# divortio/divortio-lz4

Hardware: AMD Instinct MI355X
Metric: LZ4 compress+decompress GB/s on 4 MiB independent blocks; % of HBM peak (higher is better)
Workload: dtype u8; 1 GPU; raw block decompress, 4096 x 4 MiB independent blocks per GPU (tiles216), device-resident (BASELINE.json configs[1]); blocks_per_gpu=4096, block_bytes=4194304, generator=tiles216, parallelism=blocks sharded x1

## Files before the change

### divortio-lz4_amd/csrc/lz4mi_decompress.hip

```cpp
#include "../../include/lz4mi.h"
#include "lz4mi_common.h"
#include "lz4mi_decompress.h"
#include "lz4mi_launch.h"

#ifndef LZ4MI_LL_ADAPT
#define LZ4MI_LL_ADAPT 127
#endif
#ifndef LZ4MI_ORDER
#define LZ4MI_ORDER 1
#endif
#ifndef LZ4MI_ABLATE
#define LZ4MI_ABLATE 0
#endif

#ifndef LZ4MI_TIMELINE
#define LZ4MI_TIMELINE 0
#endif

#ifndef LZ4MI_PROFILE
#define LZ4MI_PROFILE 0
#endif

namespace lz4mi {

// ... 686 lines not shown
        for (int k = lane; 16 * k < e0 - s0 + 20; k += kWave) {
            const int32_t q = s0 + 16 * k;
            uint4 v;
            if (q + 16 <= per) {
                v = load16<R_HIST>(c, S, R.src + q);
            } else {
                unsigned __int128 x = 0;
#pragma unroll 1
                for (int j = 0; j < 16; ++j) x |= (unsigned __int128)src[(q + j) % per] << (8 * j);
                __builtin_memcpy(&v, &x, 16);
            }
            B.w[4 * k] = v.x;
            B.w[4 * k + 1] = v.y;
            B.w[4 * k + 2] = v.z;
            B.w[4 * k + 3] = v.w;
        }
        __syncthreads();
        const int32_t a0 = (int32_t)((0u - (uint32_t)(uintptr_t)(c.dst + R.y)) & 15u);
        if (lane == 0 && a0) {
            const int32_t ph = 0 - s0;
            if ((uint32_t)ph < (uint32_t)(e0 - s0)) out16(c.dst + R.y, stage16(B.w, ph));
        }
        const int32_t np = (R.n - a0 + 15) >> 4;
        const int32_t step = (16 * kWave) % per;
        int32_t r = (a0 + 16 * lane) % per;
#pragma unroll 2
        for (int32_t p = lane; p < np; p += kWave) {
            const int32_t d0 = a0 + 16 * p;
            const bool last = d0 > dl;
            const int32_t d = last ? dl : d0;
            const int32_t ph = (last ? d % per : r) - s0;
            if ((uint32_t)ph < (uint32_t)(e0 - s0) && LZ4MI_ABLATE != 4) {
                out16(c.dst + R.y + d, stage16(B.w, ph));
            }
            r += step;
            if (r >= per) r -= per;
        }
    }
    __syncthreads();
}


__device__ __forceinline__ void long_literals(uint8_t* dst, const uint8_t* src, int32_t n, int lane) {
    const int32_t np = (n + 15) >> 4;
    auto at = [&](int32_t p) { return 16 * p < n - 16 ? 16 * p : n - 16; };
#if LZ4MI_LL_ADAPT
    const unsigned int* lat = &g_lat_active[32 * xcc_id()];
#endif
    for (int32_t p0 = lane; p0 < np; p0 += kWave * 4) {
#if LZ4MI_LL_ADAPT
        const uint32_t busy = __hip_atomic_load(lat, __ATOMIC_RELAXED, __HIP_MEMORY_SCOPE_AGENT);
#endif
        const int32_t d0 = at(p0), d1 = at(p0 + kWave), d2 = at(p0 + 2 * kWave), d3 = at(p0 + 3 * kWave);
        uint4 v0, v1, v2, v3;
        v0 = ld16_nt(src + d0);
        v1 = ld16_nt(src + d1);
        v2 = ld16_nt(src + d2);
        v3 = ld16_nt(src + d3);
        st16_nt(dst + d0, v0);
        st16_nt(dst + d1, v1);
        st16_nt(dst + d2, v2);
        st16_nt(dst + d3, v3);
#if LZ4MI_LL_ADAPT
        if (busy) __builtin_amdgcn_s_sleep(LZ4MI_LL_ADAPT);
#endif
    }
}

__device__ __forceinline__ void wave_run(const Ctx& c, DecShared& S, int lane, const Run& R, PatBuf B) {
    if (R.kind == R_NONE || R.n <= 0) return;
    const bool in_buf = R.kind == R_HIST || (R.kind == R_BYTES && c.out_off + R.src >= 0);
    if (in_buf && R.period && R.n > kPeriodBulk &&
        B.bytes > 0 && (R.period + 48 <= B.bytes || (R.n >= 4 * R.period && B.bytes >= 1024))) {
        periodic_run(c, S, lane, R, B);
        return;
    }
    const int np = run_pieces(R.n);
    if (R.kind == R_BYTES) {
        for (int p = lane; p < np; p += kWave) {
            const Piece P = plan_piece(R, p);
            bytes_piece(c, P.y, P.a, P.b, P.w, P.period);
        }
        return;
    }
    if (R.period) {
        WaveGen<kWaveB2> g{R, np, 0, lane};
        pipe<R_HIST, true, kWaveB2>(c, S, g);
        return;
    }
    WaveGen<kWaveB> g{R, np, 0, lane};
    if (R.kind == R_LDS) pipe<R_LDS, false, kWaveB>(c, S, g);
    else if (R.kind == R_COMP && R.n >= kLongLit) long_literals(c.dst + R.y, c.blk + R.src, R.n, lane);
    else if (R.kind == R_COMP) pipe<R_COMP, false, kWaveB>(c, S, g);
    else pipe<R_HIST, false, kWaveB>(c, S, g);
}

__device__ __forceinline__ void short_literals(const Ctx& c, int32_t y, int32_t n, const uint4& v) {
    if (LZ4MI_ABLATE == 4) return;
    uint8_t* d = c.dst + y;
    uint64_t lo = v.x | ((uint64_t)v.y << 32);
    const uint64_t hi = v.z | ((uint64_t)v.w << 32);
    int32_t o = 0;
    if (n & 8) { __builtin_memcpy(d, &lo, 8); lo = hi; o = 8; }
    if (n & 4) { const uint32_t t = (uint32_t)lo; __builtin_memcpy(d + o, &t, 4); lo >>= 32; o += 4; }
    if (n & 2) { const uint16_t t = (uint16_t)lo; __builtin_memcpy(d + o, &t, 2); lo >>= 16; o += 2; }
    if (n & 1) d[o] = (uint8_t)lo;
}

constexpr int kLitRuns = 64;
constexpr int kLitRows = kLitRuns * (kLaneBytes / 16) / 64;
static_assert((kChunk + 16) / 17 <= kLitRuns, "every run of >= 16 literal bytes of a chunk has a list entry");
static_assert(kLim / 16 + kLitRuns <= 3 * 64, "a chunk's own runs: at most three piece rows");
static_assert(kLim / 16 + kLitRuns <= kLitRows * 64, "... which the bitmap holds");
static_assert(kLitRuns * sizeof(PEnt) + kLitRows * 8 <= sizeof(uint32_t) * kMaxSeq, "run list and bitmap fit S.pms");
static_assert(kLitRows <= kWave, "one lane clears each bitmap word");
static_assert(offsetof(DecShared, pms) % 16 == 0, "16-byte aligned list entries");

struct LitDeal {
    uint32_t P = 0, R = 0;
    static __device__ __forceinline__ PEnt* list(DecShared& S) { return reinterpret_cast<PEnt*>(S.pms); }
    static __device__ __forceinline__ uint64_t* bitmap(DecShared& S) {
        return reinterpret_cast<uint64_t*>(reinterpret_cast<uint8_t*>(S.pms) + kLitRuns * sizeof(PEnt));
    }
    __device__ __forceinline__ void add(DecShared& S, int lane, bool has, uint64_t bal, int32_t y, int32_t src, int32_t n) {
        if (R == 0) {
            if (lane < kLitRows) bitmap(S)[lane] = 0;
            __syncthreads();
        }
        const uint32_t np = has ? (uint32_t)(n + 15) >> 4 : 0u;
        const uint32_t incl = wave_incl_scan(np, lane);
        const uint32_t r = R + __builtin_amdgcn_mbcnt_hi((uint32_t)(bal >> 32), __builtin_amdgcn_mbcnt_lo((uint32_t)bal, 0u));
        const uint32_t p0 = P + incl - np;
        if (has) {
            list(S)[r] = PEnt{y, src, n, (int32_t)p0};
            atomicOr((unsigned long long*)&bitmap(S)[p0 >> 6], 1ull << (p0 & 63u));
        }
        P += lane_of(incl, kWave - 1);
        R += (uint32_t)__popcll(bal);
    }
    __device__ __forceinline__ void flush(const Ctx& c, DecShared& S, int lane) {
        if (R == 0) return;
        __syncthreads();
        const PEnt* L = list(S);
        const uint64_t* bm = bitmap(S);
        int32_t rb = -1;
        for (uint32_t t = 0; 64u * t < P; ++t) {
            const uint64_t w = bm[t];
            const int32_t below = (int32_t)__builtin_amdgcn_mbcnt_hi((uint32_t)(w >> 32), __builtin_amdgcn_mbcnt_lo((uint32_t)w, 0u));
            const int32_t r = rb + below + (int32_t)((w >> lane) & 1u);
            rb += __popcll(w);
            const uint32_t p = 64u * t + (uint32_t)lane;
            if (p < P) {
                const PEnt e = L[r];
                const int32_t d0 = 16 * ((int32_t)p - e.p0);
                const int32_t d = d0 < e.n - 16 ? d0 : e.n - 16;
                const uint4 v = stage16(S.stage, e.src + d);
                if (LZ4MI_ABLATE != 4) out16(c.dst + e.y + d, v);
            }
        }
        __syncthreads();
        P = R = 0;
    }
};

__device__ __forceinline__ void dealt_literals(const Ctx& c, DecShared& S, int lane, uint32_t nseq) {
    LitDeal D;
    for (uint32_t i = 0; 64 * i < nseq; ++i) {
        const uint32_t k = 64 * i + lane;
        const uint4& e = S.t_seq[k < nseq ? k : 0u];
        const uint32_t y = e.x, lw = e.y;
        const uint32_t n = k < nseq ? lw >> 16 : 0u;
        const bool has = n >= 16;
        const uint64_t bal = __ballot(has);
        if (bal) D.add(S, lane, has, bal, (int32_t)y, (int32_t)(lw & 0xFFFFu), (int32_t)n);
    }
    D.flush(c, S, lane);
}

__device__ __forceinline__ int64_t wave_varint(const Ctx& c, int lane, int64_t& q) {
    int64_t sum = 0;
    for (;;) {
        int64_t p = q + 16 * lane;
        int first = 16;
        uint32_t lastb = 0;
        for (int j = 0; j < 16; ++j) {
            int64_t r = p + j;
            uint32_t b = (r < c.in_len) ? c.blk[r] : 0u;
            if (b != 255u && first == 16) { first = j; lastb = b; }
        }
        uint64_t mask = __ballot(first < 16);
        if (mask) {
            int fl = __builtin_ctzll(mask);
            int fi = lane_of(first, fl);
            uint32_t fb = lane_of(lastb, fl);
            int64_t cnt = (int64_t)fl * 16 + fi;
            sum += 255 * cnt + fb;
            q += cnt + 1;
            return sum;
        }
        sum += 255 * 16 * kWave;
        q += 16 * kWave;
    }
}

__device__ __forceinline__ uint32_t seq_error(const Ctx& c, int64_t out_start, int64_t lit, int64_t ll, uint32_t off,
                                              int64_t ml) {
    if (out_start + ll > c.cap) return 1;
    if (lit + ll > c.in_len) return 2;
    if (ml == 0) return 0;
    if (off == 0) return 3;
    int64_t ms_abs = c.out_off + out_start + ll;
    if ((int64_t)off > ms_abs + c.dict_len) return 4;
    if (c.isolate && (int64_t)off > out_start + ll) return 5;
    return 0;
}

__device__ __forceinline__ int32_t err_status(uint32_t e) { return e == 5 ? -9 : -(int32_t)e; }
template <bool XP>
__device__ __forceinline__ uint32_t seq_err(const Ctx& c, bool rel, int64_t out_start, int64_t lit, int64_t ll,
                                            uint32_t off, int64_t ml) {
    if (XP && rel) {
        if (lit + ll > c.in_len) return 2;
        if (ml == 0) return 0;
        return off == 0 ? 3u : 0u;
    }
    return seq_error(c, out_start, lit, ll, off, ml);
}

__device__ __forceinline__ uint32_t f1_changes(const Ctx& c, int32_t ms, int32_t off, int32_t ml) {
    if (ml == 0 || ml >= 8 || off < 8 || c.out_off + ms - off < 0) return 0;
    const int32_t p0 = ms + ml - 8;
    if (p0 - off < 0) return c.isolate ? 2u : 1u;
    for (int32_t p = p0; p < ms && p < c.cap; ++p)
        if (hist_u8(c.dst + p) != hist_u8(c.dst + p - off)) return 1;
    return 0;
}

__device__ __noinline__ void f1_fixup(const Ctx c, const DecShared& S, int lane, uint32_t nseq, bool cut, int64_t cut_ms,
                         int32_t coff, int32_t cml) {
    int64_t lo = INT64_MAX;
    const uint32_t n = nseq + (cut ? 1u : 0u);
    for (uint32_t k = 0; k < n; ++k) {
        int64_t ms;
        int32_t off, ml;
        if (k < nseq) {
            const SeqInfo q = seq_info(S, k);
            ms = (int64_t)q.out + q.ll;
            off = q.off;
            ml = q.ml;
        } else {
            ms = cut_ms;
            off = coff;
            ml = cml;
        }
        if (ml == 0) continue;
        const bool internal = c.out_off + ms - off >= 0;
        if (ms - off + ml > lo) {
            if (internal) {
                for (int32_t t = lane; t < ml; t += kWave) {
                    const int64_t d = ms + t;
                    const int64_t s = ms - off + (off < ml ? t % off : t);
                    const uint32_t v = hist_u8(c.dst + s);
                    if (d < c.cap) c.dst[d] = (uint8_t)v;
                }
            } else if (lane == 0) {
                for (int32_t t = 0; t < ml; ++t) {
                    const uint32_t v = hist_byte(c, ms - off + t);
                    if (ms + t < c.cap) c.dst[ms + t] = (uint8_t)v;
                }
            }
            wait_vmem();
        }
        if (internal && off >= 8 && ml < 8) {
            const int64_t p = ms + ml - 8 + lane;
            const bool mine = lane < 8 - ml && c.out_off + p >= 0 && p < c.cap;
            const uint32_t v = mine ? (c.out_off + p - off >= 0 ? hist_u8(c.dst + p - off) : 0u) : 0u;
            if (mine) c.dst[p] = (uint8_t)v;
            const int64_t p0 = ms + ml - 8;
            if (p0 < lo) lo = p0;
            wait_vmem();
        }
    }
}

__device__ __forceinline__ int32_t stored_block(const DecArgs& a, const Ctx& c, uint32_t b, uint32_t out_cap, int lane) {
    int32_t status = 0;
    const int32_t n = c.in_len;
    if ((uint32_t)n > out_cap) {
        status = LZ4MI_ERR_RANGE_STATUS;
    } else if (n >= 16) {
        long_literals(c.dst, c.blk, n, lane);
    } else if (lane < n) {
        c.dst[lane] = c.blk[lane];
    }
    if (lane == 0) {
        a.status[b] = status;
        a.out_len[b] = status ? 0u : (uint32_t)n;
    }
    return status;
}

struct XState {
    bool on = false;
    uint4* xs = nullptr;
    SegRec* xr = nullptr;
    uint32_t seg_lo = 0, seg_hi = 0;
    bool started = false, done = false, fail = false;
    uint32_t G = 0, X = 0, nx = 0, olen = 0, err = 0xFFFFFFFFu, entry = 0;
    int64_t OG = 0;
    int pass = 0, restart = 0;
};

template <bool LK>
__device__ __forceinline__ bool x_enter(const DecArgs& a, Ctx& c, XState& x, int lane, uint32_t wblk, uint32_t sg,
                                        uint32_t nseg, uint32_t out_cap) {
    x.on = LK || ((uint32_t)c.in_len <= a.x_in_max && out_cap <= a.x_out_max &&
                  (uint64_t)out_cap < (uint64_t)c.in_len * kXRatioMax &&
                  !(a.x_flat1 && (uint64_t)c.in_len * 16 >= (uint64_t)out_cap * 15));
    if (!x.on) return a.xphase == 0 && sg == wblk % nseg;
    const SegGeom G = seg_geom((uint32_t)c.in_len);
    if (sg >= G.S) return false;
    x.seg_lo = sg * G.L;
    x.seg_hi = sg + 1 == G.S ? (uint32_t)c.in_len : min((uint32_t)c.in_len, x.seg_lo + G.L);
    x.xs = a.xseq + (size_t)wblk * a.xseq_stride + (size_t)sg * G.stride;
    x.xr = a.xrec + (size_t)wblk * nseg + sg;
    SegRec* const xr = x.xr;
    if (a.xphase == 2) {
// ... 287 lines not shown
        if (k < nseq) {
            const SeqInfo q = seq_info(S, k);
            e = seq_err<XP>(c, rel, c.O + (uint32_t)(q.out - (int32_t)c.O), (int64_t)c.ip + q.lit, q.ll, q.off, q.ml);
        }
        first_err = wave_min(e ? (k << 3) | e : 0xFFFFFFFFu);
    }
    return SeqTable{nseq, (int64_t)carry, first_err, false};
}

struct CutSeq {
    int64_t cq = 0, cll = 0, cml = 0, clit = 0;
    uint32_t coff = 0;
};

__device__ __forceinline__ void advance(Ctx& c, int64_t tab_hi, const Parse& P, const CutSeq& cs) {
    c.O = tab_hi;
    if (P.cut) {
        c.O += cs.cll + cs.cml;
        c.ip = (int32_t)(cs.cq < c.in_len ? cs.cq : c.in_len);
    } else if (P.tail >= kEnd) {
        c.ip = c.in_len;
    } else {
        c.ip += (int32_t)P.tail;
    }
}

__device__ __forceinline__ void x_export_chunk(Ctx& c, const DecShared& S, XState& x, int lane, const Parse& P,
                                               const SeqTable& T, const CutSeq& cs) {
    const bool cut = P.cut;
    const uint32_t nseq = T.nseq, seg_lo = x.seg_lo, seg_hi = x.seg_hi;
    const int64_t tab_hi = c.O + T.total;
    const uint32_t ipc = (uint32_t)c.ip;
    const uint32_t ntot = nseq + (cut ? 1u : 0u);
    const uint32_t ecut = cut ? seq_err<true>(c, true, tab_hi, cs.clit, cs.cll, cs.coff, cs.cml) : 0u;
    const uint32_t ferr = T.first_err != 0xFFFFFFFFu ? T.first_err : (ecut ? ((nseq << 3) | ecut) : 0xFFFFFFFFu);
    const uint32_t fk = ferr == 0xFFFFFFFFu ? ntot : (ferr >> 3);
    auto x_tok = [&](uint32_t k) -> uint32_t {
        if (k >= nseq) return ipc + P.last_tok;
        const SeqInfo q = seq_info(S, k);
        return ipc + (uint32_t)q.lit - 1u - (q.ll >= 15 ? (uint32_t)(q.ll - 15) / 255u + 1u : 0u);
    };
    auto x_out = [&](uint32_t k) -> int64_t { return k >= nseq ? tab_hi : (int64_t)S.t_seq[k].x; };
    uint32_t k0 = ntot, k1 = ntot;
    for (uint32_t r = 0; 64u * r < ntot; ++r) {
        const uint32_t k = 64u * r + lane;
        const uint32_t t = k < ntot ? x_tok(k) : 0xFFFFFFFFu;
        const uint64_t m0 = __ballot(k < ntot && t >= seg_lo), m1 = __ballot(k < ntot && t >= seg_hi);
        if (k0 == ntot && m0) k0 = 64u * r + (uint32_t)__builtin_ctzll(m0);
        if (k1 == ntot && m1) k1 = 64u * r + (uint32_t)__builtin_ctzll(m1);
    }
    bool restart = false;
    if (!x.started && fk < k0) {
        if (x.pass == 0 && x.restart < kSegRestarts) {
            restart = true;
            ++x.restart;
        } else {
            x.fail = x.done = true;
        }
    } else {
        if (!x.started && k0 < ntot) {
            x.started = true;
            x.G = x_tok(k0);
            x.OG = x_out(k0);
        }
        if (x.started) {
            const uint32_t ke = fk < k1 ? fk + 1 : k1;
            for (uint32_t k = k0 + lane; k < ke; k += kWave) {
                uint4 e;
                if (k < nseq) {
                    const SeqInfo q = seq_info(S, k);
                    e = make_uint4((uint32_t)(x_out(k) - x.OG), ipc + (uint32_t)q.lit, (uint32_t)q.ll,
                                   q.ml ? (uint32_t)q.off : 0u);
                } else {
                    e = make_uint4((uint32_t)(tab_hi - x.OG), (uint32_t)cs.clit, (uint32_t)cs.cll,
                                   cs.cml ? cs.coff : 0u);
                }
                x.xs[x.nx + (k - k0)] = e;
            }
            if (fk < k1) {
                x.err = ((x.nx + (fk - k0)) << 3) | (ferr & 7u);
                x.done = true;
            } else if (k1 < ntot) {
                x.done = true;
                x.X = x_tok(k1);
                x.olen = (uint32_t)(x_out(k1) - x.OG);
            }
            x.nx += ke - k0;
        }
    }
    if (restart) {
        c.ip = (int32_t)(x_tok(fk) + 1u);
        c.O = 0;
    } else if (!x.done) {
        advance(c, tab_hi, P, cs);
        if ((uint32_t)c.ip >= seg_hi && c.ip < c.in_len) {
            if (!x.started) {
                x.started = true;
                x.G = (uint32_t)c.ip;
                x.OG = c.O;
            }
            x.done = true;
            x.X = (uint32_t)c.ip;
            x.olen = (uint32_t)(c.O - x.OG);
        }
    }
    __syncthreads();
}

__device__ __forceinline__ void x_finish(const DecArgs& a, const Ctx& c, XState& x, int lane, uint32_t sg) {
    if (!x.done) {
        if (!x.started) {
            x.G = (uint32_t)c.in_len;
            x.OG = c.O;
        }
        x.X = (uint32_t)c.in_len;
        x.olen = (uint32_t)(c.O - x.OG);
    }
    if (lane == 0) {
        SegRec* const xr = x.xr;
        xr->entry = x.G;
        xr->exit = x.X;
        xr->cnt = x.nx;
        xr->olen = x.olen;
        xr->err = x.err;
        xr->fail = (x.fail || (a.xforce && sg > 0 && (a.xforce == 2 ? x.pass != 1 : x.pass == 0))) ? 1u : 0u;
        if (x.pass == 1)
            __hip_atomic_store(&xr->fin, (x.err != 0xFFFFFFFFu ? kFinErr : x.X) + 1u, __ATOMIC_RELEASE,
                               __HIP_MEMORY_SCOPE_AGENT);
    }
}

__device__ __forceinline__ uint32_t source_map(const Ctx& c, DecShared& S, int lane, uint32_t nseq, int64_t total) {
    uint32_t msh = total >= 32u * nseq ? 5u : 4u;
    while ((total >> msh) >= kLim) ++msh;
    for (uint32_t k = lane; k < nseq; k += kWave) {
        const uint32_t t0 = S.t_seq[k].x - (uint32_t)c.O;
        const uint32_t t1 = (k + 1 < nseq ? S.t_seq[k + 1].x : (uint32_t)(c.O + total)) - (uint32_t)c.O;
        for (uint32_t b = (t0 + (1u << msh) - 1) >> msh; (b << msh) < t1; ++b) S.nxt[b] = (uint16_t)k;
    }
    __syncthreads();
    return msh;
}

__device__ __forceinline__ uint32_t round1(const Ctx& c, DecShared& S, int lane, uint32_t nseq, uint32_t msh, Prof& prof) {
    uint32_t pend = 0;
    uint32_t ready = 0;
    uint32_t rbits = 0;
    uint32_t nlit_pack = 0;
    dealt_literals(c, S, lane, nseq);
    LitDeal D;
    for (uint32_t i = 0; 64 * i < nseq; ++i) {
        const uint32_t k = 64 * i + lane;
        Run M = no_run(), ML = no_run();
        SeqInfo q = seq_info(S, k < nseq ? k : 0u);
        if (k >= nseq) q.ll = 0;
        {
            const bool shortL = q.ll > 0 && q.ll < 16;
            if (__ballot(shortL)) {
                if (shortL) short_literals(c, q.out, q.ll, stage16(S.stage, q.lit));
            }
        }
        PROF(23);
        if (k < nseq) {
            const int32_t t0 = q.out;
            M = match_run(c, t0 + q.ll, q.off, q.ml);
            if (M.n == 0) {
                M.kind = R_NONE;
            } else if (match_src_end(M) > (int32_t)c.O) {
                int32_t rs = M.src, re = match_src_end(M), li = 0, nl = 0;
                const int r = (M.kind == R_HIST && M.period == 0)
                                  ? remap_src(c, S, nseq, msh, rs, re, li, nl, i < 4)
                                  : 0;
                if (r == 3) {
                    ML = Run{M.y, nl, li, 0, R_LDS};
                    M.y += nl;
                    M.n -= nl;
                    nlit_pack |= (uint32_t)nl << (8 * i);
                }
                if (r == 1 || r == 3) {
                    M.src = rs;
                    if (c.out_off + rs < 16) M.kind = R_BYTES;
                    S.t_seq[k].w = (uint32_t)rs + (r == 3 ? kSplitBase : kMemoBase);
                    rbits |= 1u << i;
                } else if (r == 2) {
                    ML = Run{M.y, M.n, li, 0, R_LDS};
                    M.kind = R_NONE;
                } else {
                    pend |= 1u << i;
                    M.kind = R_NONE;
                }
            }
        }
        const bool longM = M.kind != R_NONE && M.n > kLaneBytes;
        const bool longML = ML.n > kLaneBytes;
        const bool fastM = M.kind == R_HIST && M.period == 0 && M.n >= 16;
        if (M.kind != R_NONE && !longM && fastM) ready |= 1u << i;
        PROF(16);
        {
            const bool dealML = ML.n >= 16 && !longML, shortML = ML.n > 0 && ML.n < 16;
            if (const uint64_t bal = __ballot(dealML)) {
                if (D.R + (uint32_t)__popcll(bal) > (uint32_t)kLitRuns) D.flush(c, S, lane);
                D.add(S, lane, dealML, bal, ML.y, ML.src, ML.n);
            }
            if (__ballot(shortML)) {
                if (shortML) short_literals(c, ML.y, ML.n, stage16(S.stage, ML.src));
            }
        }
        PROF(17);
        for (uint64_t lm = __ballot(longML); lm; lm &= lm - 1) wave_run(c, S, lane, shfl_run(ML, __builtin_ctzll(lm)), no_pat());
        if (M.kind != R_NONE && !longM && !fastM) lane_slow_run(c, S, M);
        if (const uint64_t mm0 = __ballot(longM)) {
            D.flush(c, S, lane);
            for (uint64_t mm = mm0; mm; mm &= mm - 1) wave_run(c, S, lane, shfl_run(M, __builtin_ctzll(mm)), pat_round1(S));
        }
        PROF(18);
    }
    D.flush(c, S, lane);
    piece_pipe(c, S, ready, rbits, lane, nseq, nlit_pack);
    return pend;
}

__device__ __forceinline__ void later_rounds(const Ctx& c, DecShared& S, int lane, uint32_t nseq, uint32_t pend,
                                             Prof& prof) {
    for (; LZ4MI_ABLATE != 6;) {
        uint32_t np = 0;
        for (uint32_t i = 0; 64 * i < nseq; ++i) {
            const bool pk = (pend >> i) & 1u;
            const uint64_t bal = __ballot(pk);
            if (pk) {
                const uint32_t k = 64 * i + lane;
                const uint32_t idx = np + __builtin_amdgcn_mbcnt_hi((uint32_t)(bal >> 32),
                                                                    __builtin_amdgcn_mbcnt_lo((uint32_t)bal, 0u));
                const SeqInfo q = seq_info(S, k);
                const int32_t ms = q.out + q.ll;
                S.pms[idx] = (uint32_t)ms;
                S.pme[idx] = (uint32_t)(q.ml > c.cap - ms ? c.cap : ms + q.ml);
            }
            np += (uint32_t)__popcll(bal);
        }
        if (np == 0) break;
        PROF_COUNT(11, 1);
        __syncthreads();
        wait_vmem();
        PROF(20);
        uint32_t ready = 0;
        for (uint32_t i = 0; 64 * i < nseq; ++i) {
            if (__ballot((pend >> i) & 1u) == 0) continue;
            Run M = no_run();
            if ((pend >> i) & 1u) {
                const uint32_t k = 64 * i + lane;
                const SeqInfo q = seq_info(S, k);
                M = match_run(c, q.out + q.ll, q.off, q.ml);
                const int32_t rs = M.src, re = match_src_end(M);
                uint32_t lo = 0, hi = np;
                while (lo < hi) {
                    const uint32_t mid = (lo + hi) >> 1;
                    if ((int32_t)S.pme[mid] > rs) hi = mid;
                    else lo = mid + 1;
                }
                if (lo >= np || (int32_t)S.pms[lo] >= re) pend &= ~(1u << i);
                else M.kind = R_NONE;
            }
            const bool longM = M.kind != R_NONE && M.n > kLaneBytes;
            const bool fastM = M.kind == R_HIST && M.period == 0 && M.n >= 16;
            if (M.kind != R_NONE && !longM && fastM) ready |= 1u << i;
            if (M.kind != R_NONE && !longM && !fastM) lane_slow_run(c, S, M);
            for (uint64_t mm = __ballot(longM); mm; mm &= mm - 1) wave_run(c, S, lane, shfl_run(M, __builtin_ctzll(mm)), pat_rounds(S));
        }
        piece_pipe(c, S, ready, 0u, lane, nseq, 0u);
        __syncthreads();
    }
}

__device__ __forceinline__ void output_rounds(const Ctx& c, DecShared& S, int lane, const SeqTable& T, Prof& prof) {
    const uint32_t msh = source_map(c, S, lane, T.nseq, T.total);
    PROF(22);
    const uint32_t pend = round1(c, S, lane, T.nseq, msh, prof);
    PROF(19);
    later_rounds(c, S, lane, T.nseq, pend, prof);
}

__device__ __forceinline__ int32_t f1_table(const Ctx& c, const DecShared& S, int lane, uint32_t nseq) {
    bool cand = false;
    for (uint32_t k = lane; k < nseq; k += kWave) {
        const SeqInfo q = seq_info(S, k);
        cand |= q.ml != 0 && q.ml < 8 && q.off >= 8;
    }
    if (__ballot(cand)) {
        wait_vmem();
        uint32_t dv = 0;
        for (uint32_t k = lane; k < nseq; k += kWave) {
            const SeqInfo q = seq_info(S, k);
            dv |= f1_changes(c, q.out + q.ll, q.off, q.ml);
        }
        if (__ballot(dv & 2u)) return -9;
        if (__ballot(dv)) f1_fixup(c, S, lane, nseq, false, 0, 0, 0);
    }
    return 0;
}

__device__ __forceinline__ int32_t cut_match(const Ctx& c, DecShared& S, int lane, int32_t ms, const CutSeq& cs,
                                             bool f1check) {
    const Run M = match_run(c, ms, (int32_t)cs.coff, (int32_t)cs.cml);
    if (M.n > 0) {
        wait_vmem();
        wave_run(c, S, lane, M, pat_all(S));
    }
    if (f1check && cs.cml != 0 && cs.cml < 8 && cs.coff >= 8) {
        wait_vmem();
        const uint32_t dv = lane == 0 ? f1_changes(c, ms, (int32_t)cs.coff, (int32_t)cs.cml) : 0u;
        if (__ballot(dv & 2u)) return -9;
        if (__ballot(dv)) f1_fixup(c, S, lane, 0, true, (int64_t)ms, (int32_t)cs.coff, (int32_t)cs.cml);
    }
    return 0;
}

constexpr bool kOutput = LZ4MI_ABLATE == 0 || LZ4MI_ABLATE >= 4;
constexpr bool kParseOnly = LZ4MI_ABLATE == 2 || LZ4MI_ABLATE == 3;

template <bool XP, bool LK = false, bool CH = false>
__device__ __forceinline__ int32_t decompress_block(const DecArgs& a, uint32_t cblk = 0, uint64_t cbase = 0) {
    __shared__ DecShared S;
    const int lane = threadIdx.x;
    const uint32_t nseg = XP ? a.xsegs : 1u;
    if (!CH && blockIdx.x >= a.nblocks * nseg) return 0;
    const uint32_t wblk = CH ? cblk : XP ? blockIdx.x / nseg : blockIdx.x;
    const uint32_t sg = XP ? blockIdx.x - wblk * nseg : 0u;
    if (LK && uniform(a.xcnt[wblk]) == kNotExported) return 0;
    const uint32_t b = CH ? cblk : a.order ? uniform(a.order[wblk]) : wblk;
    if (!CH && !XP && a.redo && !uniform(a.redo[b])) return 0;
#if LZ4MI_TIMELINE
    const uint64_t tl_t0 = wall_clock64();
#endif
    const uint64_t in_off = uniform64(a.in_off[b]), out_off = uniform64(a.out_off[b]);
    const uint32_t out_cap = uniform(a.out_cap[b]);
    Ctx c;
    c.blk = a.in + in_off;
    const uint32_t word = uniform(a.in_len[b]);
    c.in_len = (int32_t)(a.frame_words ? word & 0x7FFFFFFFu : word);
    c.out_off = CH ? (int64_t)(out_off - cbase) : (int64_t)out_off;
    c.dst = a.out + out_off;
    c.cap = out_cap > 0x7FFFFFFFu ? 0x7FFFFFFF : (int32_t)out_cap;
    c.dict = a.dict;
    c.dict_len = a.dict ? (int32_t)a.dict_len : 0;
    c.isolate = a.isolate;
    c.ip = 0;
    c.O = 0;
    if (a.frame_words && (word & 0x80000000u)) {
        return stored_block(a, c, b, out_cap, lane);
    }
    XState x;
    if constexpr (XP) {
        if (!x_enter<LK>(a, c, x, lane, wblk, sg, nseg, out_cap)) return 0;
    }
    const bool xp = XP && x.on;
#if LZ4MI_LL_ADAPT
    const bool lat_bound = (uint64_t)c.in_len * 2 < (uint64_t)out_cap;
    unsigned int* lat = &g_lat_active[32 * xcc_id()];
    if (lat_bound && lane == 0) atomicAdd(lat, 1u);
#endif
    Prefetch pf;
    Prof prof;
#if LZ4MI_PROFILE
    prof = Prof{{0}, (uint64_t)wall_clock64()};
#endif
    int32_t status = 0;
    while (c.ip < c.in_len) {
        if (XP && x.done) break;
        PROF_COUNT(10, 1);
        stage_chunk(c, S, pf, lane);
        const uint32_t rem = (uint32_t)(c.in_len - c.ip);
        Parse P;
        SeqTable T;
        for (bool fast_tab = rem > kFastRem;; fast_tab = false) {
            P = parse_chunk(S, lane, rem, fast_tab, !XP, prof);
            if (LZ4MI_ABLATE != 3 && !P.cut && P.tail < kEnd && (int64_t)c.ip + P.tail < c.in_len)
                prefetch(c, pf, (int64_t)c.ip + P.tail, lane);
            if (kParseOnly) break;
            T = seq_table<XP>(c, S, lane, rem, xp, fast_tab, P, prof);
            if (!T.redo) break;
            wait_vmem();
            settle(pf);
            __syncthreads();
        }
        if (kParseOnly) {
            c.ip = P.tail == kEnd ? c.in_len : c.ip + (P.cut ? kChunk : (int32_t)P.tail);
            __syncthreads();
            continue;
        }
        if (T.first_err != 0xFFFFFFFFu && !xp) { status = err_status(T.first_err & 7); break; }
        PROF(3);
        CutSeq cs;
        {
            const uint8_t* s = (const uint8_t*)S.stage;
            int64_t cq = 0, cll = 0, cml = 0, clit = 0;
            uint32_t coff = 0;
            if (P.cut) {
                constexpr uint32_t kStaged = 16 * (kStageWords / 4);
                uint32_t r = P.last_tok;
                const uint32_t tok = s[r++];
                cll = tok >> 4;
                bool more = cll == 15;
                while (more && r < kStaged) {
                    const uint32_t b = s[r++];
                    cll += b;
                    more = b == 255;
                }
                int64_t q = (int64_t)c.ip + r;
                if (more) cll += wave_varint(c, lane, q);
                clit = q;
                q += cll;
                if (q < c.in_len) {
                    uint32_t w[4];
                    if (q + 16 <= c.in_len) {
                        __builtin_memcpy(w, c.blk + q, 16);
                    } else {
                        const uint4 t = load16_tail(c.blk, q, c.in_len);
                        w[0] = t.x;
                        w[1] = t.y;
                        w[2] = t.z;
                        w[3] = t.w;
                    }
                    coff = w[0] & 0xFFFFu;
                    q += 2;
                    cml = tok & 15;
                    if (cml == 15) {
                        bool run = true;
                        for (int t = 2; t < 16 && run; ++t) {
                            const uint32_t wd = t < 4 ? w[0] : t < 8 ? w[1] : t < 12 ? w[2] : w[3];
                            const uint32_t b = (wd >> (8 * (t & 3))) & 255u;
                            cml += b;
                            ++q;
                            run = b == 255;
                        }
                        if (run) cml += wave_varint(c, lane, q);
                    }
                    cml += 4;
                }
                cq = q;
            }
            cs = CutSeq{cq, cll, cml, clit, coff};
        }
        if constexpr (XP) {
            if (xp) {
                x_export_chunk(c, S, x, lane, P, T, cs);
                continue;
            }
        }
        const int64_t tab_hi = c.O + T.total;
        if (P.cut && cs.cq < c.in_len) prefetch(c, pf, cs.cq, lane);
        if (kOutput) {
            PROF(4);
            __builtin_amdgcn_s_setprio(3);
            wait_vmem();
            settle(pf);
            PROF(21);
            output_rounds(c, S, lane, T, prof);
            PROF(6);
        }
        if (P.cut) {
            if (kOutput) PROF_COUNT(12, 1);
            const uint32_t e = seq_error(c, tab_hi, cs.clit, cs.cll, cs.coff, cs.cml);
            if (e) { status = err_status(e); break; }
            if (kOutput)
                wave_run(c, S, lane, Run{(int32_t)tab_hi, (int32_t)cs.cll, (int32_t)cs.clit, 0, cs.cll ? (uint32_t)R_COMP : (uint32_t)R_NONE}, no_pat());
        }
        PROF(7);
        if (a.f1check) {
            status = f1_table(c, S, lane, T.nseq);
            if (status) break;
        }
        if (kOutput && P.cut) {
            status = cut_match(c, S, lane, (int32_t)(tab_hi + cs.cll), cs, a.f1check);
            if (status) break;
        }
        advance(c, tab_hi, P, cs);
        __syncthreads();
        PROF(8);
    }
    if constexpr (XP) {
        if (xp) {
            x_finish(a, c, x, lane, sg);
#if LZ4MI_LL_ADAPT
            if (lat_bound && lane == 0) atomicSub(lat, 1u);
#endif
            return 0;
        }
    }
#if LZ4MI_PROFILE
    if (lane == 0)
        for (int i = 0; i < 24; ++i) atomicAdd(&g_prof[i], (unsigned long long)prof.acc[i]);
#endif
    if (lane == 0) {
        a.status[b] = status;
        a.out_len[b] = status ? 0u : (uint32_t)c.O;
        if (XP) a.xcnt[b] = kNotExported;
    }
#if LZ4MI_LL_ADAPT
    if (lat_bound && lane == 0) atomicSub(lat, 1u);
#endif
#if LZ4MI_TIMELINE
    wait_vmem();
    const uint64_t tl_t1 = wall_clock64();
    uint32_t hw, xcc;
    asm volatile("s_getreg_b32 %0, hwreg(HW_REG_HW_ID)" : "=s"(hw));
    asm volatile("s_getreg_b32 %0, hwreg(HW_REG_XCC_ID)" : "=s"(xcc));
    if (lane == 0 && b < kTlMax) {
        g_tl[2 * b] = tl_t0;
        g_tl[2 * b + 1] = tl_t1;
        g_tl_id[2 * b] = hw;
        g_tl_id[2 * b + 1] = xcc;
    }
#endif
    return status;
}

__global__ __launch_bounds__(64, 4) void lz4mi_decompress_kernel(DecArgs a) { (void)decompress_block<false>(a); }
__global__ __launch_bounds__(64, 4) void lz4mi_decompress_x_kernel(DecArgs a) { (void)decompress_block<true>(a); }
__global__ __launch_bounds__(64, 4) void lz4mi_decompress_xl_kernel(DecArgs a) { (void)decompress_block<true, true>(a); }

__global__ __launch_bounds__(64) void lz4mi_xverify_kernel(DecArgs a) {
    static_assert(kSegMax == 4 * 64, "four records per lane");
    const uint32_t b = blockIdx.x, lane = threadIdx.x;
    if (a.xcnt[b] == kNotExported) return;
    const uint32_t nseg = a.xsegs, in_len = a.in_len[b];
    const SegGeom G = seg_geom(in_len);
    SegRec* R = a.xrec + (size_t)b * nseg;
    uint32_t entry[4], exit[4], err[4], fail[4], hi_l[4], my_fin[4], kind[4];
#pragma unroll
    for (int q = 0; q < 4; ++q) {
        const uint32_t sg = 64u * q + lane;
        const bool in = sg < G.S;
        entry[q] = in ? R[sg].entry : 0u;
        exit[q] = in ? R[sg].exit : 0u;
        err[q] = in ? R[sg].err : 0xFFFFFFFFu;
        fail[q] = in ? R[sg].fail : 0u;
        hi_l[q] = sg + 1 >= G.S ? in_len : min(in_len, sg * G.L + G.L);
        my_fin[q] = 0;
        kind[q] = 0;
    }
    uint32_t pex[4], per[4];
#pragma unroll
    for (int q = 0; q < 4; ++q) {
        pex[q] = __shfl_up(exit[q], 1);
        per[q] = __shfl_up(err[q], 1);
        if (lane == 0) {
            pex[q] = q ? __builtin_amdgcn_readlane(exit[q > 0 ? q - 1 : 0], 63) : 0u;
            per[q] = q ? __builtin_amdgcn_readlane(err[q > 0 ? q - 1 : 0], 63) : 0xFFFFFFFFu;
        }
    }
    uint32_t s0 = G.S;
#pragma unroll
    for (int q = 3; q >= 0; --q) {
        const uint32_t sg = 64u * q + lane;
        const bool ok = sg < G.S && (sg == 0 || (!fail[q] && entry[q] == pex[q] && per[q] == 0xFFFFFFFFu &&
                                                 pex[q] < hi_l[q]));
        const uint64_t bad = __ballot(sg < G.S && !ok);
        if (bad) s0 = 64u * q + (uint32_t)__builtin_ctzll(bad);
    }
#pragma unroll
    for (int q = 0; q < 4; ++q)
        if (64u * q + lane < s0) my_fin[q] = err[q] != 0xFFFFFFFFu ? kFinErr : exit[q];
    uint32_t first = G.S, prev = 0;
    if (s0 > 0 && s0 < G.S) {
        const uint32_t t = s0 - 1;
        uint32_t v = 0;
#pragma unroll
        for (int q = 0; q < 4; ++q)
            if ((t >> 6) == (uint32_t)q) v = __builtin_amdgcn_readlane(my_fin[q], t & 63);
        prev = v;
    }
    bool stop = s0 >= G.S;
#pragma unroll
    for (int q = 0; q < 4; ++q) {
        if (stop || 64u * q + 63 < s0) continue;
        for (uint32_t l = 64u * q < s0 ? s0 - 64u * q : 0u; l < 64 && !stop; ++l) {
            const uint32_t sg = 64u * q + l;
            if (sg >= G.S) {
                stop = true;
                break;
            }
            const uint32_t hi = __builtin_amdgcn_readlane(hi_l[q], l);
            const uint32_t en = __builtin_amdgcn_readlane(entry[q], l), ex = __builtin_amdgcn_readlane(exit[q], l);
            const uint32_t er = __builtin_amdgcn_readlane(err[q], l), fl = __builtin_amdgcn_readlane(fail[q], l);
            uint32_t fin, k = 0;
            if (sg > 0 && prev == kFinErr) {
                fin = kFinErr;
                k = 1;
            } else if (sg > 0 && prev >= hi) {
                fin = prev;
                k = 1;
            } else if (sg == 0 || (!fl && en == prev)) {
                fin = er != 0xFFFFFFFFu ? kFinErr : ex;
            } else {
                first = sg;
                stop = true;
                break;
            }
            if (lane == l) {
                my_fin[q] = fin;
                kind[q] = k;
            }
            prev = fin;
        }
    }
#pragma unroll
    for (int q = 0; q < 4; ++q) {
        const uint32_t sg = 64u * q + lane;
        if (sg < first) {
            if (kind[q]) {
                if (my_fin[q] != kFinErr) R[sg].entry = R[sg].exit = my_fin[q];
                R[sg].cnt = 0;
                R[sg].olen = 0;
                R[sg].err = 0xFFFFFFFFu;
            }
            R[sg].fin = my_fin[q] + 1u;
        }
    }
    if (lane == 0) a.xfirst_w[b] = first;
#pragma unroll
    for (int q = 0; q < 4; ++q) {
        const uint32_t sg = 64u * q + lane;
        const bool redo = sg < G.S && sg >= first && sg > 0 && (fail[q] || entry[q] != pex[q]) &&
                          per[q] == 0xFFFFFFFFu && pex[q] >= sg * G.L && pex[q] < hi_l[q];
        if (sg < G.S) R[sg].from = redo ? pex[q] : kNoBase;
    }
}

constexpr uint32_t kOrderMax = 8192;
__global__ __launch_bounds__(1024) void lz4mi_block_order_kernel(const uint32_t* in_len, const uint32_t* out_cap,
                                                                 uint32_t n, uint32_t* order) {
    __shared__ uint64_t key[kOrderMax];
    const uint32_t t = threadIdx.x;
    uint32_t m = 2;
    while (m < n) m <<= 1;
    for (uint32_t i = t; i < m; i += 1024) {
        uint64_t k = ~0ull;
        if (i < n) {
            const uint32_t il = in_len[i], oc = out_cap[i];
            const bool lat = (uint64_t)il * 2 < (uint64_t)oc;
            const uint32_t work = LZ4MI_ORDER == 2 ? 0u : (il > 0x7FFFFFFFu ? 0x7FFFFFFFu : il);
            const uint32_t hi = lat ? 0x7FFFFFFFu - work : 0x80000000u;
            k = ((uint64_t)hi << 32) | i;
        }
        key[i] = k;
    }
    __syncthreads();
    for (uint32_t size = 2; size <= m; size <<= 1) {
        for (uint32_t stride = size >> 1; stride > 0; stride >>= 1) {
            for (uint32_t i = t; i < (m >> 1); i += 1024) {
                const uint32_t lo = 2 * i - (i & (stride - 1)), hi = lo + stride;
                const bool asc = (lo & size) == 0;
                const uint64_t x = key[lo], y = key[hi];
                if ((x > y) == asc) {
                    key[lo] = y;
                    key[hi] = x;
                }
            }
            __syncthreads();
        }
    }
    for (uint32_t i = t; i < n; i += 1024) order[i] = (uint32_t)key[i];
}

__global__ __launch_bounds__(64, 4) void lz4mi_decompress_frames_chain_kernel(DecArgs a, const int64_t* finfo,
                                                                              const uint64_t* frame_out_off,
                                                                              uint32_t nframes) {
    const int lane = threadIdx.x;
    const uint32_t f = blockIdx.x;
    if (f >= nframes) return;
    const int64_t* fi = finfo + 8ull * f;
    if (uniform64((uint64_t)fi[0]) || uniform64((uint64_t)fi[7])) return;
    const uint64_t first = uniform64((uint64_t)fi[4]), n = uniform64((uint64_t)fi[6]);
    if (first > a.nblocks || n > a.nblocks - first) return;
    const uint64_t base = uniform64(frame_out_off[f]);
    uint64_t k = 0;
    if ((uniform64((uint64_t)fi[1]) & 0x20) || n < 2) {
        uint64_t hit = 0;
        for (; k < n && !hit; k += kWave) {
            const uint64_t q = k + lane;
            hit = __ballot(q < n && a.status[first + q] == LZ4MI_ERR_CROSS_BLOCK);
        }
        if (!hit) return;
        k = k - kWave + (uint64_t)__builtin_ctzll(hit);
    }
    bool failed = false;
    for (; k < n; ++k) {
        const uint32_t b = (uint32_t)(first + k);
        if (failed) {
            if (lane == 0) {
                a.status[b] = LZ4MI_ERR_CROSS_BLOCK;
                a.out_len[b] = 0;
            }
            continue;
        }
        failed = uniform((uint32_t)decompress_block<false, false, true>(a, b, base)) != 0;
        wait_vmem();
        __syncthreads();
    }
}

}

#if LZ4MI_PROFILE
extern "C" int lz4mi_debug_prof(unsigned long long* out) {
    if (hipMemcpyFromSymbol(out, HIP_SYMBOL(lz4mi::g_prof), sizeof(unsigned long long) * 24) != hipSuccess) return -1;
    unsigned long long z[24] = {0};
    return hipMemcpyToSymbol(HIP_SYMBOL(lz4mi::g_prof), z, sizeof z) == hipSuccess ? 0 : -1;
}
#endif

#if LZ4MI_TIMELINE
extern "C" int lz4mi_debug_timeline(unsigned long long* t, unsigned int* id, unsigned int n) {
    if (n > lz4mi::kTlMax) n = lz4mi::kTlMax;
    if (hipMemcpyFromSymbol(t, HIP_SYMBOL(lz4mi::g_tl), sizeof(unsigned long long) * 2 * n) != hipSuccess) return -1;
    return hipMemcpyFromSymbol(id, HIP_SYMBOL(lz4mi::g_tl_id), sizeof(unsigned int) * 2 * n) == hipSuccess ? 0 : -1;
}
#endif

using lz4mi::Batch;
using lz4mi::DecArgs;
using lz4mi::XLayout;

static DecArgs dec_args(const Batch& b, int isolate, int f1check) {
    return DecArgs{b.in, b.in_off, b.in_len, b.out, b.out_off, b.out_cap, b.dict, b.dict_len, b.out_len, b.status,
                   b.nblocks, isolate, f1check};
}

extern "C" hipError_t lz4mi_launch_decompress(const Batch& b, int mode, int isolate, uint32_t* order,
                                              hipStream_t stream) {
    const int fw = (mode & 4) ? 1 : 0;
    mode &= 3;
    const uint32_t nblocks = b.nblocks;
    DecArgs a = dec_args(b, isolate, mode == 2 ? 1 : 0);
    a.frame_words = fw;
    if (nblocks == 0) return hipSuccess;
    if (mode == 1) return lz4mi_launch_decompress_serial(a, stream);
    if (LZ4MI_ORDER && order && nblocks > 1 && nblocks <= lz4mi::kOrderMax) {
        hipLaunchKernelGGL(lz4mi::lz4mi_block_order_kernel, dim3(1), dim3(1024), 0, stream, b.in_len, b.out_cap,
                           nblocks, order);
        a.order = order;
    }
    hipLaunchKernelGGL(lz4mi::lz4mi_decompress_kernel, dim3(nblocks), dim3(64), 0, stream, a);
    return hipGetLastError();
}

extern "C" hipError_t lz4mi_launch_decompress_frames_chain(const Batch& b, int mode, const int64_t* finfo,
                                                           const uint64_t* frame_out_off, uint32_t nframes,
                                                           hipStream_t stream) {
    if (nframes == 0 || b.nblocks == 0) return hipSuccess;
    DecArgs a = dec_args(b, 0, mode == 2 ? 1 : 0);
    a.dict = nullptr;
    a.dict_len = 0;
    a.frame_words = 1;
    hipLaunchKernelGGL(lz4mi::lz4mi_decompress_frames_chain_kernel, dim3(nframes), dim3(64), 0, stream, a, finfo,
                       frame_out_off, nframes);
    return hipGetLastError();
}

using lz4mi::kSegMax;
extern "C" size_t lz4mi_small_scratch_bytes(uint32_t nblocks, uint32_t x_in_max, uint32_t x_out_max) {
    return lz4mi::x_layout(nblocks, x_in_max, x_out_max, false).total;
}
extern "C" size_t lz4mi_linked_scratch_bytes(uint32_t nblocks, uint32_t x_in_max, uint32_t x_out_max) {
    return lz4mi::x_layout(nblocks, x_in_max, x_out_max, true).total;
}

static hipError_t zero_parse_meta(const XLayout& L, void* xs, hipStream_t stream) {
    return hipMemsetAsync(L.xcnt.in<uint8_t>(xs), 0, L.ptr.off - L.xcnt.off, stream);
}
static hipError_t parse_exported(DecArgs a, const XLayout& L, void* xs, int force_reparse, void (*kernel)(DecArgs),
                                 hipStream_t stream) {
    a.xseq = L.xseq.in<uint4>(xs);
    a.xcnt = L.xcnt.in<uint32_t>(xs);
    a.xrec = L.xrec.in<lz4mi::SegRec>(xs);
    a.xseq_stride = L.stride;
    a.xsegs = kSegMax;
    a.x_in_max = L.x_in_max;
    a.x_out_max = L.x_out_max;
    a.xfirst = L.xfirst.in<uint32_t>(xs);
    a.xfirst_w = L.xfirst.in<uint32_t>(xs);
    a.xforce = force_reparse;
    const dim3 grid(a.nblocks * kSegMax);
    hipLaunchKernelGGL(kernel, grid, dim3(64), 0, stream, a);
    hipLaunchKernelGGL(lz4mi::lz4mi_xverify_kernel, dim3(a.nblocks), dim3(64), 0, stream, a);
    a.xphase = 2;
    hipLaunchKernelGGL(kernel, grid, dim3(64), 0, stream, a);
    hipLaunchKernelGGL(lz4mi::lz4mi_xverify_kernel, dim3(a.nblocks), dim3(64), 0, stream, a);
    a.xphase = 1;
    hipLaunchKernelGGL(kernel, grid, dim3(64), 0, stream, a);
    return hipGetLastError();
}

extern "C" hipError_t lz4mi_launch_decompress_small(const Batch& b, uint32_t x_in_max, uint32_t x_out_max, void* xs,
                                                    int force_reparse, int f1, hipStream_t stream) {
    const uint32_t nblocks = b.nblocks;
    if (nblocks == 0) return hipSuccess;
    const XLayout L = lz4mi::x_layout(nblocks, x_in_max, x_out_max, false);
    hipError_t e = zero_parse_meta(L, xs, stream);
    if (e != hipSuccess) return e;
    DecArgs a = dec_args(b, nblocks > 1 ? 1 : 0, f1);
    a.x_flat1 = nblocks >= 64 ? 1 : 0;
    e = parse_exported(a, L, xs, force_reparse, lz4mi::lz4mi_decompress_x_kernel, stream);
    if (e != hipSuccess) return e;
    e = lz4mi_launch_expand(b, L, xs, false, f1, 0, stream);
    if (e != hipSuccess || !f1) return e;
    DecArgs r = dec_args(b, nblocks > 1 ? 1 : 0, 1);
    r.redo = L.redo.in<uint32_t>(xs);
    hipLaunchKernelGGL(lz4mi::lz4mi_decompress_kernel, dim3(nblocks), dim3(64), 0, stream, r);
    return hipGetLastError();
}

extern "C" hipError_t lz4mi_launch_decompress_linked(const Batch& b, uint32_t x_in_max, uint32_t x_out_max, void* xs,
                                                     int force_reparse, int frame_words, int has_prev, int f1,
                                                     hipStream_t stream) {
    if (b.nblocks == 0) return hipSuccess;
    const XLayout L = lz4mi::x_layout(b.nblocks, x_in_max, x_out_max, true);
    hipError_t e = zero_parse_meta(L, xs, stream);
    if (e == hipSuccess) e = lz4mi_launch_linked_prep(b, L, xs, frame_words, has_prev, stream);
    if (e != hipSuccess) return e;
    DecArgs a = dec_args(b, 0, 0);
    a.in_len = L.head.in<uint32_t>(xs) + 8;
    e = parse_exported(a, L, xs, force_reparse, lz4mi::lz4mi_decompress_xl_kernel, stream);
    if (e != hipSuccess) return e;
    return lz4mi_launch_expand(b, L, xs, true, f1, frame_words, stream);
}
```

Baseline: 1597 GB/s.

## Specialize decompress kernel on f1check and route short literals through deal

```diff
diff --git a/divortio-lz4_amd/csrc/lz4mi_decompress.hip b/divortio-lz4_amd/csrc/lz4mi_decompress.hip
--- a/divortio-lz4_amd/csrc/lz4mi_decompress.hip
+++ b/divortio-lz4_amd/csrc/lz4mi_decompress.hip
@@ -862,10 +862,14 @@
             const uint32_t p = 64u * t + (uint32_t)lane;
             if (p < P) {
                 const PEnt e = L[r];
-                const int32_t d0 = 16 * ((int32_t)p - e.p0);
-                const int32_t d = d0 < e.n - 16 ? d0 : e.n - 16;
-                const uint4 v = stage16(S.stage, e.src + d);
-                if (LZ4MI_ABLATE != 4) out16(c.dst + e.y + d, v);
+                if (e.n < 16) {
+                    short_literals(c, e.y, e.n, stage16(S.stage, e.src));
+                } else {
+                    const int32_t d0 = 16 * ((int32_t)p - e.p0);
+                    const int32_t d = d0 < e.n - 16 ? d0 : e.n - 16;
+                    const uint4 v = stage16(S.stage, e.src + d);
+                    if (LZ4MI_ABLATE != 4) out16(c.dst + e.y + d, v);
+                }
             }
         }
         __syncthreads();
@@ -880,9 +884,12 @@
         const uint4& e = S.t_seq[k < nseq ? k : 0u];
         const uint32_t y = e.x, lw = e.y;
         const uint32_t n = k < nseq ? lw >> 16 : 0u;
-        const bool has = n >= 16;
+        const bool has = n >= 16, shortL = n > 0 && n < 16;
         const uint64_t bal = __ballot(has);
         if (bal) D.add(S, lane, has, bal, (int32_t)y, (int32_t)(lw & 0xFFFFu), (int32_t)n);
+        if (__ballot(shortL)) {
+            if (shortL) short_literals(c, (int32_t)y, (int32_t)n, stage16(S.stage, (int32_t)(lw & 0xFFFFu)));
+        }
     }
     D.flush(c, S, lane);
 }
@@ -1476,14 +1483,7 @@
     for (uint32_t i = 0; 64 * i < nseq; ++i) {
         const uint32_t k = 64 * i + lane;
         Run M = no_run(), ML = no_run();
-        SeqInfo q = seq_info(S, k < nseq ? k : 0u);
-        if (k >= nseq) q.ll = 0;
-        {
-            const bool shortL = q.ll > 0 && q.ll < 16;
-            if (__ballot(shortL)) {
-                if (shortL) short_literals(c, q.out, q.ll, stage16(S.stage, q.lit));
-            }
-        }
+        const SeqInfo q = seq_info(S, k < nseq ? k : 0u);
         PROF(23);
         if (k < nseq) {
             const int32_t t0 = q.out;
@@ -1521,13 +1521,10 @@
         if (M.kind != R_NONE && !longM && fastM) ready |= 1u << i;
         PROF(16);
         {
-            const bool dealML = ML.n >= 16 && !longML, shortML = ML.n > 0 && ML.n < 16;
+            const bool dealML = ML.n > 0 && !longML;
             if (const uint64_t bal = __ballot(dealML)) {
                 if (D.R + (uint32_t)__popcll(bal) > (uint32_t)kLitRuns) D.flush(c, S, lane);
                 D.add(S, lane, dealML, bal, ML.y, ML.src, ML.n);
-            }
-            if (__ballot(shortML)) {
-                if (shortML) short_literals(c, ML.y, ML.n, stage16(S.stage, ML.src));
             }
         }
         PROF(17);
@@ -1642,9 +1639,11 @@
 constexpr bool kOutput = LZ4MI_ABLATE == 0 || LZ4MI_ABLATE >= 4;
 constexpr bool kParseOnly = LZ4MI_ABLATE == 2 || LZ4MI_ABLATE == 3;
 
-template <bool XP, bool LK = false, bool CH = false>
+constexpr int kF1Arg = -1, kF1Off = 0, kF1On = 1;
+template <bool XP, bool LK = false, bool CH = false, int F1 = kF1Arg>
 __device__ __forceinline__ int32_t decompress_block(const DecArgs& a, uint32_t cblk = 0, uint64_t cbase = 0) {
     __shared__ DecShared S;
+    const bool f1check = F1 == kF1Arg ? a.f1check != 0 : F1 == kF1On;
     const int lane = threadIdx.x;
     const uint32_t nseg = XP ? a.xsegs : 1u;
     if (!CH && blockIdx.x >= a.nblocks * nseg) return 0;
@@ -1790,12 +1789,12 @@
                 wave_run(c, S, lane, Run{(int32_t)tab_hi, (int32_t)cs.cll, (int32_t)cs.clit, 0, cs.cll ? (uint32_t)R_COMP : (uint32_t)R_NONE}, no_pat());
         }
         PROF(7);
-        if (a.f1check) {
+        if (f1check) {
             status = f1_table(c, S, lane, T.nseq);
             if (status) break;
         }
         if (kOutput && P.cut) {
-            status = cut_match(c, S, lane, (int32_t)(tab_hi + cs.cll), cs, a.f1check);
+            status = cut_match(c, S, lane, (int32_t)(tab_hi + cs.cll), cs, f1check);
             if (status) break;
         }
         advance(c, tab_hi, P, cs);
@@ -1839,7 +1838,12 @@
     return status;
 }
 
-__global__ __launch_bounds__(64, 4) void lz4mi_decompress_kernel(DecArgs a) { (void)decompress_block<false>(a); }
+__global__ __launch_bounds__(64, 4) void lz4mi_decompress_kernel(DecArgs a) {
+    (void)decompress_block<false, false, false, kF1Off>(a);
+}
+__global__ __launch_bounds__(64, 4) void lz4mi_decompress_ref_kernel(DecArgs a) {
+    (void)decompress_block<false, false, false, kF1On>(a);
+}
 __global__ __launch_bounds__(64, 4) void lz4mi_decompress_x_kernel(DecArgs a) { (void)decompress_block<true>(a); }
 __global__ __launch_bounds__(64, 4) void lz4mi_decompress_xl_kernel(DecArgs a) { (void)decompress_block<true, true>(a); }
 
@@ -2065,7 +2069,8 @@
                            nblocks, order);
         a.order = order;
     }
-    hipLaunchKernelGGL(lz4mi::lz4mi_decompress_kernel, dim3(nblocks), dim3(64), 0, stream, a);
+    hipLaunchKernelGGL(mode == 2 ? lz4mi::lz4mi_decompress_ref_kernel : lz4mi::lz4mi_decompress_kernel, dim3(nblocks),
+                       dim3(64), 0, stream, a);
     return hipGetLastError();
 }
 
@@ -2131,7 +2136,7 @@
     if (e != hipSuccess || !f1) return e;
     DecArgs r = dec_args(b, nblocks > 1 ? 1 : 0, 1);
     r.redo = L.redo.in<uint32_t>(xs);
-    hipLaunchKernelGGL(lz4mi::lz4mi_decompress_kernel, dim3(nblocks), dim3(64), 0, stream, r);
+    hipLaunchKernelGGL(lz4mi::lz4mi_decompress_ref_kernel, dim3(nblocks), dim3(64), 0, stream, r);
     return hipGetLastError();
 }
 
```

Result: faster. 1666 GB/s (median of 6 runs) (+4.4%).
